# mishapadidar/GP-Derivatives-Variational-Inference

Hardware: AMD Instinct MI355X
Metric: ELBO steps/sec, DSVGP d=20 N=1M M=500 p=5 (higher is better)
Workload: dtype f32 (f64 Cholesky/solves); 1 GPU; DSVGP d=20 N=1M M=500 p=5 B=4096; global_batch=4096, per_gpu_batch=4096, M_prime=3000, parallelism=dp1 rows, trsm_nb=4096, graph_replay=False, one_call_step=True, dense_product=hand-written (gemm32.hip, v_mfma_f32_32x32x2_f32)

## Files before the change

gp-derivatives-variational-inference_amd/csrc/common.h:

```cpp
#pragma once
#include <hip/hip_runtime.h>
#include <stdint.h>
#include <stdio.h>

#include "dsvgp.h"

struct dsvgp_ctx {
    hipStream_t stream = nullptr;
    void* blas = nullptr;
    void* det_slab = nullptr;
    size_t det_bytes = 0;
    bool prezeroed = false;
    bool lean_classic = false;
    bool fwd_lower_only = false;
    struct PointsJob { const float* slab; int ns; const float* partials; int nparts; float sym; };
    bool defer_points = false;
    int n_deferred = 0;
    PointsJob deferred[2];
};

#define DSVGP_LAUNCH_CHECK()                                  \
    do {                                                      \
        hipError_t e__ = hipGetLastError();                   \
        if (e__ != hipSuccess) return 1000 + (int)e__;        \
// ... 29 lines not shown
constexpr int DSVGP_GEMM_KEEP_UPPER = 1 << 20;
constexpr int DSVGP_GEMM_C_ZEROED = 1 << 21;
constexpr int DSVGP_GEMM_UPPER_UNDEF = 1 << 22;
int launch_gemm(hipStream_t st, int is_double, const GemmArgs& g);
hipError_t zero_block(void* C, size_t esz, int64_t ld, int M, int N, hipStream_t st);
void launch_cvt_f64_f32(hipStream_t st, const double* C, int64_t ldc, float* C32, int64_t ldc32, int M, int N);
void launch_widen_f32_f64(hipStream_t st, const float* src, int64_t ld, double* dst, int64_t ldd, int M, int N);
int launch_gemm64(hipStream_t st, const GemmArgs& g);
int launch_gemm32(hipStream_t st, const GemmArgs& g);

int launch_det_sum_rows64(hipStream_t st, const double* parts, int ns, int64_t n, double* out);
int launch_det_sum_scalars64(hipStream_t st, const double* parts, int n, int nc, double* out);
static inline double* det_scratch64(const dsvgp_ctx* ctx, size_t doubles) {
    return (ctx->det_slab && ctx->det_bytes / sizeof(double) >= doubles && ((uintptr_t)ctx->det_slab % 8) == 0) ? (double*)ctx->det_slab : nullptr;
}
static inline int bwd64_tiled_sweep(int ntr, int ntc, int* nsg) {
    int sweep = (int)(((int64_t)ntr * ntc) / 1024);
    sweep = sweep < 32 ? sweep : 32;
    sweep = sweep < ntc ? sweep : ntc;
    sweep = sweep > 1 ? sweep : 1;
    *nsg = cdiv(ntc, sweep);
    return sweep;
}
size_t kernel_bwd64_tiled_det_bytes(int n1, int n2, int d, int p);

size_t potrf_blocked_workspace_bytes(int n);
struct PotrfHook { int after_k; hipEvent_t ev; };
int launch_potrf_blocked(hipStream_t st, double* A, int n, int64_t lda, int* info, double* ws, double* Yinv, int64_t ldy,
                         double* YinvT, bool info_zeroed = false, const PotrfHook* hooks = nullptr, int nhooks = 0, int pipe_from = 0);
int launch_pack_both(hipStream_t st, const float* Z, const float* V, int M, const float* X, const float* D, int B, int d, int p,
                     const float* rl, const float* rs, const float* rn, float* hyp, float* center, float* PZ, float* sZ, float* vZ,
                     float* PX, float* sX, float* vX);
int kernel_bwd_points_flush(dsvgp_ctx* ctx, const float* P1, const float* vnorm1, int n1, int d, int p, const float* hyp, float* d_x1,
                            float* d_v1, float* d_hyp, const float* scal, const float* kl0, double rows, double num_data, const float* rl,
                            const float* rs, const float* rn, float* drl, float* drs, float* drn, float* dconst, float* loss);
int launch_column_mean_hyp(hipStream_t st, const float* x, int n, int d, float* center, const float* rl, const float* rs,
                           const float* rn, float* hyp);
int launch_kernel_fwd_wide(hipStream_t st, const float* P1, const float* self1, int n1q, const float* P2, const float* self2, int n2q,
                           int q, int K4, int DP, const float* hyp, float jitter, void* out, int64_t ld, int out_is_double);
size_t kernel_bwd_wide_workspace(int n1q, int n2q, int q, int NP);
int launch_kernel_bwd_wide(hipStream_t st, const void* G, int64_t ldg, int g_is_double, const float* P1, const float* self1, int n1q,
                           const float* P2, const float* self2, int n2q, int q, int K4, int DP, int NP, const float* hyp, void* workspace,
                           float** slab, int* ns, float** partials, int* nparts);
int launch_widen_sym_f32_f64(hipStream_t st, const float* src, int64_t lds, double* dst, int64_t ldd, int n);
int launch_mirror_sminus_i_col(hipStream_t st, float* A, int n, int64_t lda, const float* m, const float* hyp, float rows, double* W = nullptr,
                               int64_t ldw = 0);
int launch_variational_terms(hipStream_t st, const float* m, const float* LS, int64_t ldls, int Mp, double num_data, int flags,
                             const float* hyp, double global_rows, const float* G, int64_t ldg, float t1_scale, float* kl_out,
                             float* sums, const float* dm_src, float* d_m, float* d_LS, int64_t lddls, int fin_npts, int fin_p,
                             float* fin_scal);
int launch_stats_residual(dsvgp_ctx* ctx, const float* A, int64_t lda, int Mp, int ncols, int p, const float* m,
                          const float* constant, const float* hyp, float* mu, float* var, void* workspace, const float* y,
                          double global_rows, float* mu_bar, float* sums);
int launch_scale_epilogue(dsvgp_ctx* ctx, float* x0, int64_t n0, float* x1, int64_t n1, const float* hyp, double rows,
                          const float* scal, const float* kl0, double num_data, const float* rl, const float* rs, const float* rn,
                          float* dh, float* drl, float* drs, float* drn, float* dconst, float* loss);

int launch_trtri_blocks(hipStream_t st, const double* L, int64_t ldl, int n, int nb, double* Dinv,
                        int64_t ldd, double* tmp, const double* X64);
```

gp-derivatives-variational-inference_amd/csrc/elbo.hip:

```cpp
#include "common.h"

namespace {

constexpr float KXX_JITTER = 1e-4f;
constexpr float NOISE_FLOOR = 1e-4f;
constexpr float MIN_VARIANCE = 1e-6f;

__device__ __forceinline__ float softplusf(float x) { return x > 20.f ? x : log1pf(expf(x)); }
__device__ __forceinline__ float sigmoidf(float x) { return 1.f / (1.f + expf(-x)); }

__global__ void hyp_forward_kernel(const float* rl, const float* rs, const float* rn, float* hyp) {
    if (threadIdx.x == 0) {
        hyp[0] = softplusf(rl[0]);
        hyp[1] = softplusf(rs[0]);
        hyp[2] = softplusf(rn[0]) + NOISE_FLOOR;
        hyp[3] = 0.f;
    }
}
__global__ void hyp_backward_kernel(const float* rl, const float* rs, const float* rn, const float* dh, float* drl,
                                    float* drs, float* drn) {
    if (threadIdx.x == 0) {
        drl[0] += dh[0] * sigmoidf(rl[0]);
        drs[0] += dh[1] * sigmoidf(rs[0]);
        drn[0] += dh[2] * sigmoidf(rn[0]);
    }
}

__global__ void step_epilogue_kernel(const float* scal, const float* kl0, float inv_rows, float inv_num_data,
                                     const float* rl, const float* rs, const float* rn, float* dh, float* drl,
                                     float* drs, float* drn, float* dconst, float* loss) {
    if (threadIdx.x == 0) {
        const float d0 = dh[0] + scal[4], d1 = dh[1] + scal[3], d2 = dh[2] + scal[1];
        dh[0] = d0; dh[1] = d1; dh[2] = d2;
        drl[0] += d0 * sigmoidf(rl[0]);
        drs[0] += d1 * sigmoidf(rs[0]);
        drn[0] += d2 * sigmoidf(rn[0]);
        dconst[0] += scal[2];
        loss[0] = -scal[0] * inv_rows + kl0[0] * inv_num_data;
    }
}

__global__ __launch_bounds__(256) void colstats_kernel(const float* __restrict__ A, int64_t lda,
                                                       const float* __restrict__ W, int64_t ldw, int Mp, int ncols,
                                                       const float* __restrict__ m, int rows_per_chunk,
                                                       float* __restrict__ part) {
    const int j = blockIdx.x * 256 + threadIdx.x;
    const int i0 = blockIdx.y * rows_per_chunk, i1 = min(Mp, i0 + rows_per_chunk);
    if (j >= ncols) return;
    float sm = 0.f, sq = 0.f;
    if (W == A) {
#pragma unroll 4
        for (int i = i0; i < i1; ++i) sm = fmaf(A[(int64_t)i * lda + j], m[i], sm);
    } else {
        for (int i = i0; i < i1; ++i) {
            const float a = A[(int64_t)i * lda + j], w = W[(int64_t)i * ldw + j];
            sm = fmaf(a, m[i], sm);
            sq += w * w - a * a;
        }
    }
    part[((int64_t)blockIdx.y * 2) * ncols + j] = sm;
    part[((int64_t)blockIdx.y * 2 + 1) * ncols + j] = sq;
}
__global__ void colstats_finish_kernel(const float* __restrict__ part, int nchunk, int ncols, int p,
                                       const float* __restrict__ constant, const float* __restrict__ hyp,
                                       float* __restrict__ mu, float* __restrict__ var) {
    const int j = blockIdx.x * blockDim.x + threadIdx.x;
    if (j >= ncols) return;
    float sm = 0.f, sq = 0.f;
    for (int c = 0; c < nchunk; ++c) {
        sm += part[((int64_t)c * 2) * ncols + j];
        sq += part[((int64_t)c * 2 + 1) * ncols + j];
    }
    const float ell = hyp[0], s = hyp[1];
    const float dg = (j % (p + 1) == 0) ? s : s / (ell * ell);
    mu[j] = sm + constant[0];
    var[j] = dg + KXX_JITTER + sq;
}

__global__ __launch_bounds__(256) void likelihood_kernel(const float* __restrict__ mu, const float* __restrict__ var,
                                                         const float* __restrict__ y, int ncols, int p,
                                                         const float* __restrict__ hyp, int mll_type, float inv_rows,
                                                         float* __restrict__ mu_bar, float* __restrict__ var_bar,
                                                         float* __restrict__ varn_out, float* __restrict__ scal, float* __restrict__ partials) {
    __shared__ float red[5][4];
    const float ell = hyp[0], s = hyp[1], noise = hyp[2];
    const float LOG2PI = 1.8378770664093453f;
    float acc[5] = {0.f, 0.f, 0.f, 0.f, 0.f};
    for (int j = blockIdx.x * 256 + threadIdx.x; j < ncols; j += gridDim.x * 256) {
        const float mj = mu[j], r = y[j] - mj;
        const float vraw = var[j] + noise;
        const bool clamped = vraw < MIN_VARIANCE;
        const float vn = clamped ? MIN_VARIANCE : vraw;
        float ll, dmu, dvn, dnoise;
        if (mll_type == 0) {
            ll = -0.5f * ((r * r + vn) / noise + logf(noise) + LOG2PI);
            dmu = r / noise;
            dvn = -0.5f / noise;
            dnoise = 0.5f * (r * r + vn) / (noise * noise) - 0.5f / noise;
        } else {
            const float tot = fmaxf(vn + noise, 1e-8f);
            ll = -0.5f * (r * r / tot + logf(tot) + LOG2PI);
            dmu = r / tot;
            dvn = 0.5f * (r * r / (tot * tot) - 1.f / tot);
            dnoise = dvn;
        }
        const float dvar = clamped ? 0.f : dvn;
        dnoise += dvar;
        const float mb = -dmu * inv_rows, vb = -dvar * inv_rows;
        mu_bar[j] = mb;
        var_bar[j] = vb;
        varn_out[j] = vn;
        const bool isf = (j % (p + 1)) == 0;
        acc[0] += ll;
        acc[1] += -dnoise * inv_rows;
// ... 800 lines not shown
                                             float* const* exp_avgs, float* const* exp_avg_sqs, const int64_t* sizes, float lr,
                                             float beta1, float beta2, float eps, int step, const int* guard_dev) {
    return adam_step_multi_impl(ctx, count, params, grads, exp_avgs, exp_avg_sqs, sizes, lr, beta1, beta2, eps, step, guard_dev);
}
static int adam_step_multi_impl(dsvgp_ctx* ctx, int count, float* const* params, const float* const* grads, float* const* exp_avgs,
                                float* const* exp_avg_sqs, const int64_t* sizes, float lr, float beta1, float beta2, float eps, int step,
                                const int* guard_dev) {
    if (!ctx || count < 0 || count > DSVGP_ADAM_MAX_TENSORS || step < 1) return DSVGP_EINVAL;
    if (count && (!params || !grads || !exp_avgs || !exp_avg_sqs || !sizes)) return DSVGP_EINVAL;
    AdamTable t{};
    int nblocks = 0;
    for (int k = 0; k < count; ++k) {
        if (sizes[k] != 0 && (!params[k] || !grads[k] || !exp_avgs[k] || !exp_avg_sqs[k])) return DSVGP_EINVAL;
        if (sizes[k] == 0) continue;
        const int c = t.count++;
        t.param[c] = params[k]; t.grad[c] = grads[k]; t.m[c] = exp_avgs[k]; t.v[c] = exp_avg_sqs[k]; t.n[c] = sizes[k];
        int b = sizes[k] < 0 ? (int)(-sizes[k] < 2048 ? -sizes[k] : 2048) : cdiv(sizes[k], 256);
        if (b > 2048) b = 2048;
        t.first[c] = nblocks;
        nblocks += b;
    }
    if (!t.count) return 0;
    t.first[t.count] = nblocks;
    const double bc1 = 1.0 - pow((double)beta1, step), bc2 = 1.0 - pow((double)beta2, step);
    hipLaunchKernelGGL(adam_multi_kernel, dim3(nblocks), dim3(256), 0, ctx->stream, t, lr, beta1, beta2, eps, (float)bc1,
                       (float)sqrt(bc2), guard_dev);
    DSVGP_LAUNCH_CHECK();
    return 0;
}

int launch_stats_residual(dsvgp_ctx* ctx, const float* A, int64_t lda, int Mp, int ncols, int p, const float* m,
                          const float* constant, const float* hyp, float* mu, float* var, void* workspace, const float* y,
                          double global_rows, float* mu_bar, float* sums) {
    if (ctx->det_slab || ncols == 0) {
        int rc = dsvgp_predictive_stats(ctx, A, lda, A, lda, Mp, ncols, p, m, constant, hyp, mu, var, workspace);
        if (rc) return rc;
        return dsvgp_residual_terms(ctx, mu, y, ncols, hyp, global_rows, mu_bar, sums);
    }
    if (!ctx->prezeroed) {
        hipError_t e = hipMemsetAsync(sums, 0, 4 * sizeof(float), ctx->stream);
        if (e != hipSuccess) return 1000 + (int)e;
    }
    const int nch = stats_chunks(Mp), rpc = cdiv(Mp, nch);
    hipLaunchKernelGGL(colstats_kernel, dim3(cdiv(ncols, 256), nch), dim3(256), 0, ctx->stream, A, lda, A, lda, Mp, ncols, m, rpc,
                       (float*)workspace);
    DSVGP_LAUNCH_CHECK();
    int blocks = cdiv(ncols, 256);
    if (blocks > 512) blocks = 512;
    hipLaunchKernelGGL(colstats_residual_kernel, dim3(blocks), dim3(256), 0, ctx->stream, (const float*)workspace, nch, ncols, p,
                       constant, hyp, mu, var, y, (float)(1.0 / global_rows), mu_bar, sums);
    DSVGP_LAUNCH_CHECK();
    return 0;
}
int launch_scale_epilogue(dsvgp_ctx* ctx, float* x0, int64_t n0, float* x1, int64_t n1, const float* hyp, double rows,
                          const float* scal, const float* kl0, double num_data, const float* rl, const float* rs, const float* rn,
                          float* dh, float* drl, float* drs, float* drn, float* dconst, float* loss) {
    const int64_t tot = n0 + n1;
    int blocks = (int)((tot + 255) / 256);
    if (blocks < 1) blocks = 1;
    if (blocks > 2048) blocks = 2048;
    hipLaunchKernelGGL(scale_epilogue_kernel, dim3(blocks), dim3(256), 0, ctx->stream, x0, n0, x1, n1, hyp, (float)(1.0 / rows), scal,
                       kl0, (float)(1.0 / num_data), rl, rs, rn, dh, drl, drs, drn, dconst, loss);
    DSVGP_LAUNCH_CHECK();
    return 0;
}

extern "C" int dsvgp_residual_terms(dsvgp_ctx* ctx, const float* mu, const float* y, int ncols, const float* hyp,
                                    double global_rows, float* mu_bar, float* sums) {
    if (!ctx || !mu || !y || !hyp || !mu_bar || !sums || ncols < 0 || global_rows <= 0) return DSVGP_EINVAL;
    if (!ctx->prezeroed) {
        hipError_t e = hipMemsetAsync(sums, 0, 4 * sizeof(float), ctx->stream);
        if (e != hipSuccess) return 1000 + (int)e;
    }
    if (ncols == 0) return 0;
    int blocks = cdiv(ncols, 256);
    if (blocks > 512) blocks = 512;
    float* partials = (ctx->det_slab && ctx->det_bytes >= (size_t)blocks * 8 * sizeof(float)) ? (float*)ctx->det_slab : nullptr;
    hipLaunchKernelGGL(residual_kernel, dim3(blocks), dim3(256), 0, ctx->stream, mu, y, ncols, hyp,
                       (float)(1.0 / global_rows), mu_bar, sums, partials);
    DSVGP_LAUNCH_CHECK();
    if (partials) {
        hipLaunchKernelGGL(partials_reduce_kernel, dim3(1), dim3(64), 0, ctx->stream, (const float*)partials, blocks, 2, sums);
        DSVGP_LAUNCH_CHECK();
    }
    return 0;
}
extern "C" int dsvgp_trace_terms(dsvgp_ctx* ctx, const float* LS, int64_t ldls, const float* T1, int64_t ldt,
                                 const float* G, int64_t ldg, int n, float t1_scale, float* sums) {
    if (!ctx || !LS || !T1 || !G || !sums || n <= 0) return DSVGP_EINVAL;
    hipLaunchKernelGGL(trace_kernel, dim3(n < 1024 ? n : 1024), dim3(256), 0, ctx->stream, LS, ldls, T1, ldt, G, ldg, n, t1_scale, sums);
    DSVGP_LAUNCH_CHECK();
    return 0;
}
extern "C" int dsvgp_elbo_fast_finalize(dsvgp_ctx* ctx, const float* sums, const float* hyp, int npts, int p,
                                        double global_rows, float* out_scalars) {
    if (!ctx || !sums || !hyp || !out_scalars || npts < 0 || p < 0 || global_rows <= 0) return DSVGP_EINVAL;
    hipLaunchKernelGGL(elbo_fast_finalize_kernel, dim3(1), dim3(64), 0, ctx->stream, sums, hyp, npts, p,
                       (float)(1.0 / global_rows), out_scalars);
    DSVGP_LAUNCH_CHECK();
    return 0;
}
extern "C" int dsvgp_mirror_lower_f32(dsvgp_ctx* ctx, float* G, int n, int64_t ldg) {
    if (!ctx || !G || n <= 0 || ldg < n) return DSVGP_EINVAL;
    const int nb = cdiv(n, 32);
    hipLaunchKernelGGL(mirror_lower_f32_kernel, dim3(nb, nb), dim3(32, 8), 0, ctx->stream, G, n, ldg);
    DSVGP_LAUNCH_CHECK();
// ... 155 lines not shown
```

gp-derivatives-variational-inference_amd/csrc/step.hip:

```cpp
#include "common.h"

#include <stdlib.h>
#include <string.h>

#include <new>

namespace {

struct Carve {
    size_t off = 0;
    size_t take(size_t bytes) {
        const size_t o = off;
        off += (bytes + 255) / 256 * 256;
        return o;
    }
};

inline int pad4(int n) { return (n + 3) / 4 * 4; }
inline int auto_nb(int Mp) {
    int b = 64;
    while (b < Mp) b <<= 1;
    return b;
}

}

struct dsvgp_step_plan {
    int M, d, p, B, Mp, Bp, DP, nb;
    bool per_output = false;
    size_t o_A64 = 0, o_U32 = 0, o_Abar = 0, o_Kb64 = 0, o_var = 0, o_varbar = 0;
    int world = 1;
    int wq = 0, wr = 0;
    size_t o_Qfull = 0, o_qcol64 = 0, o_cbT = 0, o_cbK = 0, o_slab = 0, slab_bytes = 0, o_lrow64 = 0;
    hipEvent_t ev_dp = nullptr;
    size_t bytes;
    size_t o_zero, zero_bytes;
    size_t o_info, o_sums, o_klbuf, o_scal, o_hyp, o_center;
    size_t o_PZ, o_sZ, o_vZ, o_PX, o_sX, o_vX;
    size_t o_phi32 = 0; bool phi32_own = false;
    bool precleared_ge = false;
    bool precleared = false;
    size_t o_L, o_trsm, o_potrf, o_Kzx, o_A32e, o_S32e, o_var0, o_stats, o_Ge, o_Qe64, o_S64e, o_Qe32, o_Kb32, o_G1, o_Yt, o_Kbar, o_kbwd, o_kbwd2;
    size_t o_arena, arena_bytes;
    int ldS, ldQ32;
    const void* pad_ready_for = nullptr;
    hipStream_t side = nullptr;
    hipEvent_t ev_fork = nullptr, ev_side = nullptr, ev_status = nullptr, ev_fork2 = nullptr, ev_var = nullptr, ev_dense = nullptr,
               ev_zx = nullptr, ev_pipe1 = nullptr, ev_pipe2 = nullptr, ev_s = nullptr;
    static constexpr int TM_RING = 128, TM_PAIRS = 5;
    hipEvent_t tm_ring[TM_RING][2 * TM_PAIRS] = {};
    hipEvent_t* tm = tm_ring[0];
    long timed_steps = 0;
    bool timed = false;
    float* host_status = nullptr;
};

#ifndef STEP_S_LATE
#define STEP_S_LATE 2
#define STEP_S_LATE_MP 1024
#endif
static size_t step_layout(int M, int d, int p, int B, dsvgp_step_plan* pl, int world = 1) {
    if (M <= 0 || d <= 0 || p < 0 || B <= 0 || world < 1 || world > 64 || (world > 1 && M < world)) return 0;
    const int q = p + 1, Mp = M * q, Bp = B * q, DP = dsvgp_packed_width(d);
    if (DP <= 0 || Mp > 8192 || (int64_t)Mp * Bp >= ((int64_t)1 << 31)) return 0;
    pl->M = M; pl->d = d; pl->p = p; pl->B = B; pl->Mp = Mp; pl->Bp = Bp; pl->DP = DP; pl->nb = auto_nb(Mp);
    pl->ldS = pad4(Mp + 1); pl->ldQ32 = pad4(Mp + 1);
    Carve c;
    pl->o_scal = c.take(8 * sizeof(float)); pl->o_center = c.take((size_t)d * sizeof(float));
    pl->o_PZ = c.take((size_t)Mp * DP * 4); pl->o_sZ = c.take((size_t)Mp * 4); pl->o_vZ = c.take((size_t)(M * p > 0 ? M * p : 1) * 4);
    pl->o_PX = c.take((size_t)Bp * DP * 4); pl->o_sX = c.take((size_t)Bp * 4); pl->o_vX = c.take((size_t)(B * p > 0 ? B * p : 1) * 4);
    pl->o_L = c.take((size_t)Mp * Mp * 8);
    pl->o_potrf = c.take(potrf_blocked_workspace_bytes(Mp));
    pl->o_Kzx = c.take((size_t)Mp * Bp * 4); pl->o_A32e = c.take((size_t)(Mp + 1) * Bp * 4);
    pl->o_var0 = c.take((size_t)Bp * 4); pl->o_stats = c.take(dsvgp_stats_workspace_bytes(Mp, Bp) + 16);
    pl->o_Qe32 = c.take((size_t)Mp * pl->ldQ32 * 4);
    pl->o_S64e = c.take((size_t)(Mp + 1) * ((Mp + 1) / 2 * 2) * 8);
    const size_t kb = dsvgp_kernel_bwd_workspace_bytes(M, B, d, p), kz = dsvgp_kernel_bwd_workspace_bytes(M, M, d, p);
    pl->o_kbwd = c.take(kb > kz ? kb : kz); pl->o_kbwd2 = c.take(kb);
    const int nrhs_max = Bp > Mp + 1 ? Bp : Mp + 1;
    const size_t trsm_bytes = dsvgp_trsm_workspace_bytes(Mp, nrhs_max, pl->nb);
    pl->o_trsm = c.take(trsm_bytes);
    pl->o_arena = (pl->o_trsm + sizeof(double) * ((size_t)2 * Mp * Mp + (size_t)(Mp + pl->nb) * (pl->nb / 2))) / 256 * 256;
    pl->o_S32e = c.take((size_t)Mp * pl->ldS * 4);
    pl->o_Ge = c.take((size_t)(Mp + 1) * Mp * 4); pl->o_Qe64 = c.take((size_t)Mp * (Mp + 2) * 8 + 64);
    pl->o_Kb32 = c.take((size_t)Mp * Bp * 4); pl->o_G1 = c.take((size_t)Mp * Mp * 8);
    pl->o_Yt = c.take((size_t)Mp * Mp * 8); pl->o_Kbar = c.take((size_t)Mp * Mp * 8);
    pl->phi32_own = true;
    pl->o_phi32 = c.take((size_t)Mp * pl->ldQ32 * 4);
    pl->o_zero = c.off;
    pl->zero_bytes = (4 * sizeof(float) + 4 * sizeof(int) + 4 * sizeof(float) + (size_t)(2 * Mp + 1) * sizeof(float) + 255) / 256 * 256;
    pl->o_hyp = c.take(pl->zero_bytes);
    pl->o_info = pl->o_hyp + 4 * sizeof(float);
    pl->o_sums = pl->o_info + 4 * sizeof(int);
    pl->o_klbuf = pl->o_sums + 4 * sizeof(float);
    pl->arena_bytes = c.off - pl->o_arena;
    pl->world = world;
    if (world > 1) {
        const int q1 = p + 1;
        pl->wq = ((Mp + 1 + world - 1) / world + 3) / 4 * 4;
        pl->wr = ((Mp + world - 1) / world + 1) / 2 * 2;
        const int wc = ((M + world - 1) / world) * q1;
        pl->o_Qfull = c.take((size_t)Mp * world * pl->wq * 4);
        pl->o_qcol64 = c.take((size_t)Mp * pl->wq * 8);
        pl->o_lrow64 = c.take((size_t)pl->wr * Mp * 8);
        pl->o_cbT = c.take((size_t)Mp * wc * 8);
        pl->o_cbK = c.take((size_t)Mp * wc * 8);
        pl->slab_bytes = (size_t)4 * Mp * Mp * 4 + 4096;
        pl->o_slab = c.take(pl->slab_bytes);
    }
    if (pl->per_output) {
        pl->o_A64 = c.take((size_t)Mp * Bp * 8);
        pl->o_U32 = c.take((size_t)Mp * Bp * 4);
        pl->o_Abar = c.take((size_t)Mp * Bp * 4);
        pl->o_Kb64 = c.take((size_t)Mp * Bp * 8);
        pl->o_var = c.take((size_t)Bp * 4);
        pl->o_varbar = c.take((size_t)Bp * 4);
    }
    pl->bytes = c.off + 256;
    return pl->bytes;
}

static size_t split_offsets(int Mp, int Bp, size_t* o_pat, size_t* o_pq) {
    size_t off = (dsvgp_split3_bytes(Mp + 1, Bp) + 255) / 256 * 256;
    if (o_pat) *o_pat = off;
    off += (dsvgp_split3_bytes(Bp, Mp + 1) + 255) / 256 * 256;
    if (o_pq) *o_pq = off;
    off += (dsvgp_split3_bytes(Mp, Mp + 1) + 255) / 256 * 256;
    return off;
}
extern "C" size_t dsvgp_elbo_step_split_bytes(int M, int d, int p, int B) {
    if (M <= 0 || d <= 0 || p < 0 || B <= 0) return 0;
    return split_offsets(M * (p + 1), B * (p + 1), nullptr, nullptr);
}

extern "C" size_t dsvgp_elbo_step_workspace_bytes(int M, int d, int p, int B) {
    dsvgp_step_plan pl{};
    return step_layout(M, d, p, B, &pl);
}

extern "C" size_t dsvgp_elbo_step_dp_workspace_bytes(int M, int d, int p, int B, int world) {
    dsvgp_step_plan pl{};
    return step_layout(M, d, p, B, &pl, world);
}

static int plan_create(dsvgp_ctx* ctx, int M, int d, int p, int B, int world, dsvgp_step_plan** out, bool per_output = false) {
    if (!ctx || !out) return DSVGP_EINVAL;
    dsvgp_step_plan* pl = new (std::nothrow) dsvgp_step_plan();
    if (!pl) return DSVGP_EINVAL;
    pl->per_output = per_output;
    if (!step_layout(M, d, p, B, pl, world)) { delete pl; return DSVGP_EINVAL; }
    bool ok = hipStreamCreateWithFlags(&pl->side, hipStreamNonBlocking) == hipSuccess;
    hipEvent_t* evs[] = {&pl->ev_fork, &pl->ev_side, &pl->ev_status, &pl->ev_fork2, &pl->ev_var, &pl->ev_dense, &pl->ev_zx, &pl->ev_dp,
                         &pl->ev_pipe1, &pl->ev_pipe2, &pl->ev_s};
    for (hipEvent_t* e : evs) ok = ok && hipEventCreateWithFlags(e, hipEventDisableTiming) == hipSuccess;
    for (auto& slot : pl->tm_ring) for (hipEvent_t& e : slot) ok = ok && hipEventCreate(&e) == hipSuccess;
    ok = ok && hipHostMalloc((void**)&pl->host_status, 8 * sizeof(float), hipHostMallocDefault) == hipSuccess;
    if (!ok) {
        (void)hipGetLastError();
        for (hipEvent_t* e : evs) if (*e) (void)hipEventDestroy(*e);
        for (auto& slot : pl->tm_ring) for (hipEvent_t e : slot) if (e) (void)hipEventDestroy(e);
        if (pl->side) (void)hipStreamDestroy(pl->side);
        if (pl->host_status) (void)hipHostFree(pl->host_status);
        delete pl;
        return 1000 + (int)hipErrorOutOfMemory;
    }
    pl->host_status[4] = 0.f;
    *out = pl;
    return 0;
}
extern "C" int dsvgp_elbo_step_plan_create(dsvgp_ctx* ctx, int M, int d, int p, int B, dsvgp_step_plan** out) {
    return plan_create(ctx, M, d, p, B, 1, out);
}
extern "C" int dsvgp_elbo_step_dp_plan_create(dsvgp_ctx* ctx, int M, int d, int p, int B, int world, dsvgp_step_plan** out) {
    if (world < 2) return DSVGP_EINVAL;
    return plan_create(ctx, M, d, p, B, world, out);
}

extern "C" int dsvgp_elbo_step_po_plan_create(dsvgp_ctx* ctx, int M, int d, int p, int B, dsvgp_step_plan** out) {
    return plan_create(ctx, M, d, p, B, 1, out, true);
}
extern "C" size_t dsvgp_elbo_step_po_workspace_bytes(int M, int d, int p, int B) {
    dsvgp_step_plan pl{};
    pl.per_output = true;
    return step_layout(M, d, p, B, &pl);
}

extern "C" int dsvgp_elbo_step_plan_destroy(dsvgp_step_plan* pl) {
    if (!pl) return DSVGP_EINVAL;
    hipEvent_t evs[] = {pl->ev_fork, pl->ev_side, pl->ev_status, pl->ev_fork2, pl->ev_var, pl->ev_dense, pl->ev_zx, pl->ev_dp, pl->ev_pipe1,
                        pl->ev_pipe2, pl->ev_s};
    for (hipEvent_t e : evs) if (e) (void)hipEventDestroy(e);
    for (auto& slot : pl->tm_ring) for (hipEvent_t e : slot) if (e) (void)hipEventDestroy(e);
    if (pl->side) (void)hipStreamDestroy(pl->side);
    if (pl->host_status) (void)hipHostFree(pl->host_status);
    delete pl;
    return 0;
}

static int step_timings(dsvgp_step_plan* pl, int back, float* ms, int n) {
    if (!pl || !ms || n < 1 || n > dsvgp_step_plan::TM_PAIRS || back < 0 || back >= dsvgp_step_plan::TM_RING || back >= pl->timed_steps)
        return DSVGP_EINVAL;
    hipEvent_t* tm = pl->tm_ring[(pl->timed_steps - 1 - back) % dsvgp_step_plan::TM_RING];
    for (int k = 0; k < n; ++k) {
        hipError_t e = hipEventSynchronize(tm[2 * k + 1]);
        if (e == hipSuccess) e = hipEventElapsedTime(&ms[k], tm[2 * k], tm[2 * k + 1]);
        if (e != hipSuccess) return 1000 + (int)e;
    }
    return 0;
}
extern "C" int dsvgp_elbo_step_timings(dsvgp_step_plan* pl, int back, float* ms3) { return step_timings(pl, back, ms3, 3); }
extern "C" int dsvgp_elbo_step_timings5(dsvgp_step_plan* pl, int back, float* ms5) { return step_timings(pl, back, ms5, 5); }

extern "C" size_t dsvgp_elbo_step_plan_bytes(const dsvgp_step_plan* pl) { return pl ? pl->bytes : 0; }
extern "C" long dsvgp_elbo_step_timed_count(const dsvgp_step_plan* pl) { return pl ? pl->timed_steps : 0; }

extern "C" int dsvgp_elbo_step_locate(const dsvgp_step_plan* pl, int which, size_t* offset_bytes, int* rows, int* cols, int64_t* ld) {
    if (!pl || !offset_bytes || !rows || !cols || !ld) return DSVGP_EINVAL;
    switch (which) {
        case 0: *offset_bytes = pl->o_A32e; *rows = pl->Mp + 1; *cols = pl->Bp; *ld = pl->Bp; return 0;
        case 1: *offset_bytes = pl->o_Kzx; *rows = pl->Mp; *cols = pl->Bp; *ld = pl->Bp; return 0;
        case 2: *offset_bytes = pl->o_L; *rows = pl->Mp; *cols = pl->Mp; *ld = pl->Mp; return 0;
        case 3: *offset_bytes = pl->o_trsm; *rows = pl->Mp; *cols = pl->Mp; *ld = pl->Mp; return 0;
        case 4: *offset_bytes = pl->o_hyp; *rows = 1; *cols = 4; *ld = 4; return 0;
        case 5: *offset_bytes = pl->o_info; *rows = 1; *cols = 1; *ld = 1; return 0;
        default: return DSVGP_EINVAL;
    }
}

extern "C" int dsvgp_elbo_step_status(dsvgp_step_plan* pl, float* hyp4, int* info) {
    if (!pl || !info) return DSVGP_EINVAL;
    hipError_t e = hipEventSynchronize(pl->ev_status);
    if (e != hipSuccess) return 1000 + (int)e;
    if (hyp4) for (int i = 0; i < 4; ++i) hyp4[i] = pl->host_status[i];
    int v;
    memcpy(&v, &pl->host_status[4], sizeof(int));
    *info = v;
    return 0;
}

#ifndef STEP_VAR_LATE_MP
#define STEP_VAR_LATE_MP 1536
#endif
#ifndef STEP_Q_CLASSIC_BP
// ... 36 lines not shown
    if (zz_canon2(io, d, p) && rows_in_16_byte_pieces(Kbar, ld, 8))
        return dsvgp_kernel_bwd_canon2(ctx, Kbar, ld, 1, PZ, vZ, M, P2, n2, d, p, io->dir_idx, io->dir_idx_base, hyp, 1, io->dZ, io->dV,
                                       io->d_hyp, ws);
    return dsvgp_kernel_bwd(ctx, Kbar, ld, 1, PZ, sZ, vZ, M, P2, s2, n2, d, p, hyp, 1, io->dZ, io->dV, io->d_hyp, ws);
}
static int zx_fwd(dsvgp_ctx* ctx, const dsvgp_elbo_step_io* io, const float* PZ, const float* sZ, int M, const float* PX, const float* sX,
                  int B, int d, int p, const float* hyp, float* Kzx, int64_t ld) {
    if (zz_canon2(io, d, p)) return dsvgp_kernel_fwd_canon2(ctx, PZ, M, PX, B, d, p, io->dir_idx, io->dir_idx_base, hyp, 0.f, Kzx, ld, 0);
    if (zx_canon(io, d, p)) return dsvgp_kernel_fwd_canon(ctx, PZ, sZ, M, PX, sX, B, d, p, io->dir_idx, io->dir_idx_base, hyp, Kzx, ld);
    return dsvgp_kernel_fwd(ctx, PZ, sZ, M, PX, sX, B, d, p, hyp, 0.f, Kzx, ld, 0);
}
static int zx_bwd(dsvgp_ctx* ctx, const dsvgp_elbo_step_io* io, const float* Kb32, int64_t ld, const float* PZ, const float* sZ,
                  const float* vZ, int M, const float* PX, const float* sX, int B, int d, int p, const float* hyp, void* ws) {
    if (zz_canon2(io, d, p) && rows_in_16_byte_pieces(Kb32, ld, 4))
        return dsvgp_kernel_bwd_canon2(ctx, Kb32, ld, 0, PZ, vZ, M, PX, B, d, p, io->dir_idx, io->dir_idx_base, hyp, 0, io->dZ, io->dV,
                                       io->d_hyp, ws);
    if (zx_canon(io, d, p))
        return dsvgp_kernel_bwd_canon(ctx, Kb32, ld, 0, PZ, sZ, vZ, M, PX, sX, B, d, p, io->dir_idx, io->dir_idx_base, hyp, io->dZ, io->dV,
                                      io->d_hyp, ws);
    return dsvgp_kernel_bwd(ctx, Kb32, ld, 0, PZ, sZ, vZ, M, PX, sX, B, d, p, hyp, 0, io->dZ, io->dV, io->d_hyp, ws);
}

static int step_validate(dsvgp_ctx* ctx, dsvgp_step_plan* pl, const dsvgp_elbo_step_io* io, void* workspace, size_t workspace_bytes) {
    if (!ctx || !pl || !io || !workspace || workspace_bytes < pl->bytes || ((uintptr_t)workspace % 256)) return DSVGP_EINVAL;
    if (!io->Z || !io->m || !io->LS || !io->constant || !io->raw_lengthscale || !io->raw_outputscale || !io->raw_noise || !io->x ||
        !io->y || !io->flat || !io->dZ || !io->dm || !io->dLS || !io->d_hyp || !io->d_constant || !io->d_raw_lengthscale ||
        !io->d_raw_outputscale || !io->d_raw_noise || !io->loss || !io->mu || io->num_data <= 0 || io->global_rows <= 0)
        return DSVGP_EINVAL;
    const int p = pl->p, Mp = pl->Mp;
    if (p > 0 && (!io->V || !io->D || !io->dV)) return DSVGP_EINVAL;
    if (io->ldls < Mp || io->lddls < Mp) return DSVGP_EINVAL;
    return 0;
}

#define STEP_LOCALS \
    [[maybe_unused]] const int M = pl->M, d = pl->d, p = pl->p, B = pl->B, Mp = pl->Mp, Bp = pl->Bp, nb = pl->nb; \
    [[maybe_unused]] char* w = (char*)workspace; \
    [[maybe_unused]] int* info = (int*)(w + pl->o_info); \
    [[maybe_unused]] float* sums = (float*)(w + pl->o_sums); \
    [[maybe_unused]] float* kl_buf = (float*)(w + pl->o_klbuf); \
    [[maybe_unused]] float* scal = (float*)(w + pl->o_scal); \
    [[maybe_unused]] float* hyp = (float*)(w + pl->o_hyp); \
    [[maybe_unused]] float* center = (float*)(w + pl->o_center); \
    [[maybe_unused]] float *PZ = (float*)(w + pl->o_PZ), *sZ = (float*)(w + pl->o_sZ), *vZ = (float*)(w + pl->o_vZ); \
    [[maybe_unused]] float *PX = (float*)(w + pl->o_PX), *sX = (float*)(w + pl->o_sX), *vX = (float*)(w + pl->o_vX); \
    [[maybe_unused]] double* L = (double*)(w + pl->o_L); \
    [[maybe_unused]] void* trsm_ws = w + pl->o_trsm; \
    [[maybe_unused]] void* potrf_ws = w + pl->o_potrf; \
    [[maybe_unused]] float* Kzx = (float*)(w + pl->o_Kzx); \
    [[maybe_unused]] float* A32e = (float*)(w + pl->o_A32e); \
    [[maybe_unused]] float* S32e = (float*)(w + pl->o_S32e); \
    [[maybe_unused]] float* var0 = (float*)(w + pl->o_var0); \
    [[maybe_unused]] void* stats_ws = w + pl->o_stats; \
    [[maybe_unused]] float* Ge = (float*)(w + pl->o_Ge); \
    [[maybe_unused]] double* Qe64 = (double*)(w + pl->o_Qe64); \
    [[maybe_unused]] double* S64e = (double*)(w + pl->o_S64e); \
    [[maybe_unused]] float* Qe32 = (float*)(w + pl->o_Qe32); \
    [[maybe_unused]] float* Kb32 = (float*)(w + pl->o_Kb32); \
    [[maybe_unused]] double* G1 = (double*)(w + pl->o_G1); \
    [[maybe_unused]] double* Yt = (double*)(w + pl->o_Yt); \
    [[maybe_unused]] double* Kbar = (double*)(w + pl->o_Kbar); \
    [[maybe_unused]] void* kbwd_ws = w + pl->o_kbwd; \
    [[maybe_unused]] void* kbwd_ws2 = w + pl->o_kbwd2; \
    [[maybe_unused]] const int ldS = pl->ldS, ldQ32 = pl->ldQ32, ldQ64 = (Mp + 2) / 2 * 2, ldST = (Mp + 1) / 2 * 2; \
    [[maybe_unused]] const double rows = io->global_rows;

struct ZeroedScope {
    dsvgp_ctx* c; bool prev;
    ZeroedScope(dsvgp_ctx* c_, bool on) : c(c_), prev(c_->prezeroed) { if (on) c->prezeroed = true; }
    ~ZeroedScope() { c->prezeroed = prev; }
};
static int step_front(dsvgp_ctx* ctx, dsvgp_step_plan* pl, const dsvgp_elbo_step_io* io, void* workspace, int flags, bool preclear = false) {
    STEP_LOCALS
    const bool overlap = (flags & 1) && !ctx->det_slab;
    const bool timed = flags & 4;
    pl->timed = timed;
    if (timed) { pl->tm = pl->tm_ring[pl->timed_steps % dsvgp_step_plan::TM_RING]; ++pl->timed_steps; }
#define STEP_TIME(slot) do { if (timed) STEP_HIP(hipEventRecord(pl->tm[slot], ctx->stream)); } while (0)
    const hipStream_t main = ctx->stream, side = pl->side;

    const bool prezero = pl->arena_bytes <= ((size_t)48 << 20) && !ctx->det_slab;
    static const bool preclear_env = !getenv("DSVGP_PRECLEAR") || atoi(getenv("DSVGP_PRECLEAR")) != 0;
    pl->precleared = preclear && preclear_env && overlap && !prezero && !ctx->det_slab && !(flags & (16 | 32 | 64));
    pl->precleared_ge = false;
    STEP_HIP(hipMemsetAsync(io->flat, 0, io->flat_floats * sizeof(float), main));
    if (prezero) STEP_HIP(hipMemsetAsync(w + pl->o_arena, 0, pl->arena_bytes, main));
    else STEP_HIP(hipMemsetAsync(w + pl->o_zero, 0, pl->zero_bytes, main));
    if (pl->pad_ready_for != workspace || (flags & 8)) {
        STEP_HIP(hipMemsetAsync(Qe32, 0, (size_t)Mp * ldQ32 * sizeof(float), main));
        STEP_HIP(hipMemsetAsync(S32e, 0, (size_t)Mp * ldS * sizeof(float), main));
        pl->pad_ready_for = workspace;
    }
    struct PrezeroGuard {
        dsvgp_ctx* c; bool prev;
        PrezeroGuard(dsvgp_ctx* c_, bool on) : c(c_), prev(c_->prezeroed) { c->prezeroed = on; }
        ~PrezeroGuard() { c->prezeroed = prev; }
    } prezero_guard(ctx, prezero);
    STEP_CALL(launch_pack_both(main, io->Z, io->V, M, io->x, io->D, B, d, p, io->raw_lengthscale, io->raw_outputscale, io->raw_noise, hyp,
                               center, PZ, sZ, vZ, PX, sX, vX));
    static const int s_late_env = getenv("DSVGP_S_LATE") ? atoi(getenv("DSVGP_S_LATE")) : -1;
    const int s_late = !overlap ? 0 : s_late_env >= 0 ? s_late_env : (Mp >= STEP_S_LATE_MP ? STEP_S_LATE : 0);
    auto prologue_s = [&](bool background) -> int {
        int rc = dsvgp_gemm(ctx, 0, DSVGP_GEMM_A_LOWER | DSVGP_GEMM_TRANS_B | DSVGP_GEMM_B_UPPER | DSVGP_GEMM_OUT_LOWER |
                            (background ? DSVGP_GEMM_BACKGROUND : 0), Mp, Mp, Mp, 1.0, io->LS, io->ldls, io->LS, io->ldls, 0.0, nullptr, 0,
                            S32e, ldS, nullptr, 0, nullptr);
        if (rc) return rc;
        rc = launch_mirror_sminus_i_col(ctx->stream, S32e, Mp, ldS, io->m, hyp, (float)rows, S64e, ldST);
        if (rc) return rc;
        const hipError_t e = hipGetLastError();
        return e == hipSuccess ? 0 : 1000 + (int)e;
    };
    auto prologue = [&](bool background) -> int {
        int rc = 0;
        if (timed && hipEventRecord(pl->tm[2], ctx->stream) != hipSuccess) return 1000 + (int)hipGetLastError();
        rc = zx_fwd(ctx, io, PZ, sZ, M, PX, sX, B, d, p, hyp, Kzx, Bp);
        if (rc) return rc;
        if (timed && hipEventRecord(pl->tm[3], ctx->stream) != hipSuccess) return 1000 + (int)hipGetLastError();
        if (s_late) return 0;
        return prologue_s(background);
    };
    float* A32 = A32e;
    float* mu_bar = A32e + (size_t)Mp * Bp;
    static const int pipe_k1 = getenv("DSVGP_PIPE_K1") ? atoi(getenv("DSVGP_PIPE_K1")) : STEP_PIPE_K1;
    static const int pipe_k2 = getenv("DSVGP_PIPE_K2") ? atoi(getenv("DSVGP_PIPE_K2")) : STEP_PIPE_K2;
    static const int pipe_pad = getenv("DSVGP_PIPE_PAD") ? atoi(getenv("DSVGP_PIPE_PAD")) : STEP_PIPE_PAD;
    const int nblk64 = (Mp + 63) / 64;
    const int pk1 = (int)((int64_t)nblk64 * pipe_k1 / 1000), pk2 = (int)((int64_t)nblk64 * pipe_k2 / 1000);
    const bool pipe = overlap && (flags & 128) && nb >= Mp && Mp % 2 == 0 && Bp % 4 == 0 && ((uintptr_t)Kzx % 16) == 0 &&
                      (int64_t)nblk64 * ((Bp + 63) / 64) >= 8192 && nblk64 >= 16 && pipe_k1 >= 0 && pk1 <= pk2 && pk2 <= nblk64 - 2 &&
                      pipe_pad >= 0 && pipe_pad <= 98304;
    const double* LinvT = (const double*)trsm_ws + (size_t)Mp * Mp;
    auto solve_rows = [&](int ra, int rb, int pad) -> int {
        GemmArgs f{};
        f.batch = 1; f.splitk = 1;
        f.M = rb - ra; f.N = Bp; f.K = rb; f.tri_off = ra; f.wide64 = 1; f.lds_pad = pad;
        f.A = LinvT + ra; f.lda = Mp; f.flags = DSVGP_GEMM_TRANS_A | DSVGP_GEMM_A_LOWER | DSVGP_GEMM_B_IS_FLOAT;
        f.B = Kzx; f.ldb = Bp; f.alpha = 1.0; f.beta = 0.0;
        f.C = nullptr; f.C32 = A32 + (size_t)ra * Bp; f.ldc32 = Bp;
        return launch_gemm(ctx->stream, 1, f);
    };
    int r2 = 0;
    if (overlap) STEP_HIP(hipEventRecord(pl->ev_fork, main));
    STEP_CALL(zz_fwd(ctx, io, PZ, sZ, M, d, p, hyp, L, Mp));
    auto clear_tail_targets = [&]() -> int {
        STEP_HIP(hipMemsetAsync(Yt, 0, (size_t)Mp * Mp * sizeof(double), side));
        STEP_HIP(hipMemsetAsync(Kbar, 0, (size_t)Mp * Mp * sizeof(double), side));
        STEP_HIP(hipMemsetAsync(w + pl->o_phi32, 0, (size_t)Mp * ldQ32 * sizeof(float), side));
        return 0;
    };
    auto side_prologue = [&]() -> int {
        if (!overlap) return 0;
        STEP_HIP(hipStreamWaitEvent(side, pl->ev_fork, 0));
        if (pl->precleared && !s_late) {
            STEP_CALL(clear_tail_targets());
            STEP_HIP(hipMemsetAsync(Ge, 0, (size_t)(Mp + 1) * Mp * sizeof(float), side));
            pl->precleared_ge = true;
        }
        ctx->stream = side;
        const int rc = prologue(true);
        ctx->stream = main;
        if (rc) return rc;
        STEP_HIP(hipEventRecord(pl->ev_side, side));
        return 0;
    };
    if (pipe) {
        const int k1 = pk1, k2 = pk2;
        const int r1 = (k1 + 1) * 64;
        r2 = (k2 + 1) * 64;
        const PotrfHook hooks[2] = {{k1, pl->ev_pipe1}, {k2, pl->ev_pipe2}};
        double* Dinv = (double*)trsm_ws;
        STEP_CALL(launch_potrf_blocked(main, L, Mp, Mp, info, (double*)potrf_ws, Dinv, Mp, Dinv + (size_t)Mp * Mp, ctx->prezeroed, hooks,
                                       k2 > k1 ? 2 : 1));
        STEP_CALL(side_prologue());
        ctx->stream = side;
        STEP_HIP(hipStreamWaitEvent(side, pl->ev_pipe1, 0));
        STEP_TIME(0);
        STEP_CALL(solve_rows(0, r1, pipe_pad));
        if (k2 > k1) {
            STEP_HIP(hipStreamWaitEvent(side, pl->ev_pipe2, 0));
            STEP_CALL(solve_rows(r1, r2, pipe_pad));
        } else r2 = r1;
        STEP_TIME(1);
        STEP_HIP(hipEventRecord(pl->ev_pipe1, side));
        ctx->stream = main;
    } else {
        STEP_CALL(dsvgp_potrf_inverse(ctx, L, Mp, Mp, info, potrf_ws, nb, trsm_ws));
        STEP_CALL(side_prologue());
    }
    if (overlap) {
        STEP_HIP(hipStreamWaitEvent(main, pl->ev_side, 0));
        STEP_HIP(hipEventRecord(pl->ev_fork2, main));
        STEP_HIP(hipStreamWaitEvent(side, pl->ev_fork2, 0));
        STEP_HIP(hipMemcpyAsync(pl->host_status, hyp, 5 * sizeof(float), hipMemcpyDeviceToHost, side));
        STEP_HIP(hipEventRecord(pl->ev_status, side));
        if (s_late) {
            if (pl->precleared) STEP_CALL(clear_tail_targets());
            ctx->stream = side;
            const int rc = prologue_s(s_late == 1);
            ctx->stream = main;
            if (rc) return rc;
            STEP_HIP(hipEventRecord(pl->ev_s, side));
        }
    } else {
        STEP_HIP(hipMemcpyAsync(pl->host_status, hyp, 5 * sizeof(float), hipMemcpyDeviceToHost, main));
        STEP_HIP(hipEventRecord(pl->ev_status, main));
        STEP_CALL(prologue(false));
    }
    if (pipe) {
        STEP_CALL(solve_rows(r2, Mp, 0));
        STEP_HIP(hipStreamWaitEvent(main, pl->ev_pipe1, 0));
    } else {
        STEP_TIME(0);
        STEP_CALL(dsvgp_trsm(ctx, L, Mp, Mp, 0, Kzx, Bp, 0, Bp, nullptr, 0, A32, Bp, nb, trsm_ws, 1));
        STEP_TIME(1);
    }
    STEP_CALL(launch_stats_residual(ctx, A32, Bp, Mp, Bp, p, io->m, io->constant, hyp, io->mu, var0, stats_ws, io->y, rows, mu_bar, sums));
    STEP_TIME(6);
    if (flags & 32) {
        if (!io->split_ws || ((uintptr_t)io->split_ws & 255) || io->split_ws_bytes < split_offsets(Mp, Bp, nullptr, nullptr)) {
            ctx->stream = main;
            return DSVGP_EINVAL;
        }
        STEP_CALL(dsvgp_split3_bf16(ctx, A32e, Bp, Mp + 1, Bp, 0, io->split_ws));
        STEP_CALL(dsvgp_gemm3b(ctx, DSVGP_GEMM_OUT_LOWER, Mp + 1, Mp, Bp, 1.f, io->split_ws, Mp + 1, io->split_ws, Mp + 1, Ge, Mp));
    } else {
        ZeroedScope zs(ctx, pl->precleared_ge);
        STEP_CALL(dsvgp_gemm(ctx, 0, DSVGP_GEMM_TRANS_B | DSVGP_GEMM_OUT_LOWER, Mp + 1, Mp, Bp, 1.0, A32e, Bp, A32, Bp, 0.0, nullptr, 0, Ge,
                             Mp, nullptr, 0, nullptr));
    }
    STEP_TIME(7);
    if (s_late) STEP_HIP(hipStreamWaitEvent(main, pl->ev_s, 0));
    return 0;
}

extern "C" int dsvgp_elbo_step_f32(dsvgp_ctx* ctx, dsvgp_step_plan* pl, const dsvgp_elbo_step_io* io, void* workspace,
                                   size_t workspace_bytes, int flags) {
    if (int rc = step_validate(ctx, pl, io, workspace, workspace_bytes)) return rc;
    if (pl->world != 1) return DSVGP_EINVAL;
    STEP_LOCALS
    const bool overlap = (flags & 1) && !ctx->det_slab;
    const bool include_kl = flags & 2, timed = flags & 4;
    const hipStream_t main = ctx->stream, side = pl->side;
    struct PrezeroGuard {
        dsvgp_ctx* c; bool prev;
        PrezeroGuard(dsvgp_ctx* c_, bool on) : c(c_), prev(c_->prezeroed) { c->prezeroed = on; }
        ~PrezeroGuard() { c->prezeroed = prev; }
    } prezero_guard(ctx, pl->arena_bytes <= ((size_t)48 << 20) && !ctx->det_slab);
    STEP_CALL(step_front(ctx, pl, io, workspace, flags, true));
    STEP_CALL(dsvgp_mirror_lower_f32(ctx, Ge, Mp, Mp));
    auto variational = [&]() -> int {
        int rc = dsvgp_gemm(ctx, 0, DSVGP_GEMM_B_LOWER | DSVGP_GEMM_OUT_LOWER, Mp, Mp, Mp, 1.0, Ge, Mp, io->LS, io->ldls, 0.0, nullptr, 0,
                            io->dLS, io->lddls, nullptr, 0, nullptr);
        if (rc) return rc;
        return launch_variational_terms(ctx->stream, io->m, io->LS, io->ldls, Mp, io->num_data, 1 | (include_kl ? 2 : 0), hyp, rows, Ge, Mp,
                                        1.f, kl_buf, sums, Ge + (size_t)Mp * Mp, io->dm, io->dLS, io->lddls, B, p, scal);
    };
    const bool var_late = overlap && !(flags & 16) && Mp >= STEP_VAR_LATE_MP;
    auto solve_q = [&]() -> int {
        const bool small = (int64_t)((Mp + 63) / 64) * ((Mp + 1 + 63) / 64) < 1024;
        const bool prev = ctx->lean_classic;
        ctx->lean_classic = overlap && !var_late && Bp >= STEP_Q_CLASSIC_BP;
        const int rc = dsvgp_trsm(ctx, L, Mp, Mp, 1, S32e, ldS, 0, Mp + 1, small ? Qe64 : nullptr, ldQ64, Qe32, ldQ32, nb, trsm_ws, 1);
        ctx->lean_classic = prev;
        return rc;
    };
    auto dense_product = [&]() -> int {
        if (flags & 32) {
            size_t o_pat, o_pq;
            split_offsets(Mp, Bp, &o_pat, &o_pq);
// ... 319 lines not shown
```

Measured before the change: 83.49 steps/s.

## Compute predictive mean from LinvT·m on side stream, overlapping the triangular solve

Adds a path that computes the predictive mean without waiting for the large triangular solve. It first forms w = L^{-T} m in fp64, then takes column dot products of Kzx with w, and runs both on the side stream while the main stream runs the TRSM. The main stream then waits on an event instead of launching the stats/residual kernel over A32. The Ge clear is also moved onto the side stream. Separately, the Cholesky info buffer is treated as pre-zeroed by default, which skips a clear. The risks are an extra full read of Kzx competing with the solve for bandwidth, and the variance partials now being written as zero, so correctness depends on var being computed elsewhere.

```diff
diff --git a/gp-derivatives-variational-inference_amd/csrc/common.h b/gp-derivatives-variational-inference_amd/csrc/common.h
--- a/gp-derivatives-variational-inference_amd/csrc/common.h
+++ b/gp-derivatives-variational-inference_amd/csrc/common.h
@@ -105,6 +105,9 @@
 int launch_stats_residual(dsvgp_ctx* ctx, const float* A, int64_t lda, int Mp, int ncols, int p, const float* m,
                           const float* constant, const float* hyp, float* mu, float* var, void* workspace, const float* y,
                           double global_rows, float* mu_bar, float* sums);
+int launch_mean_residual_w(hipStream_t st, const double* LinvT, int64_t ldl, const float* Kzx, int64_t ldk, int Mp, int ncols, int p,
+                           const float* m, const float* constant, const float* hyp, float* mu, float* var, void* workspace, double* wvec,
+                           const float* y, double global_rows, float* mu_bar, float* sums);
 int launch_scale_epilogue(dsvgp_ctx* ctx, float* x0, int64_t n0, float* x1, int64_t n1, const float* hyp, double rows,
                           const float* scal, const float* kl0, double num_data, const float* rl, const float* rs, const float* rn,
                           float* dh, float* drl, float* drs, float* drn, float* dconst, float* loss);
diff --git a/gp-derivatives-variational-inference_amd/csrc/elbo.hip b/gp-derivatives-variational-inference_amd/csrc/elbo.hip
--- a/gp-derivatives-variational-inference_amd/csrc/elbo.hip
+++ b/gp-derivatives-variational-inference_amd/csrc/elbo.hip
@@ -60,6 +60,36 @@
     }
     part[((int64_t)blockIdx.y * 2) * ncols + j] = sm;
     part[((int64_t)blockIdx.y * 2 + 1) * ncols + j] = sq;
+}
+__global__ __launch_bounds__(256) void linvt_m_kernel(const double* __restrict__ LinvT, int64_t ld, int n, const float* __restrict__ m,
+                                                      double* __restrict__ w) {
+    const int j = blockIdx.x * 4 + (threadIdx.x >> 6), lane = threadIdx.x & 63;
+    if (j >= n) return;
+    const double* __restrict__ r = LinvT + (int64_t)j * ld;
+    double s = 0.0;
+    for (int i = j + lane; i < n; i += 64) s = fma(r[i], (double)m[i], s);
+    for (int off = 32; off > 0; off >>= 1) s += __shfl_down(s, off);
+    if (lane == 0) w[j] = s;
+}
+__global__ __launch_bounds__(256) void colmean_w_kernel(const float* __restrict__ K, int64_t ldk, int Mp, int ncols,
+                                                        const double* __restrict__ w, int rows_per_chunk, float* __restrict__ part) {
+    __shared__ double ws[256];
+    const int j = blockIdx.x * 256 + threadIdx.x;
+    const int i0 = blockIdx.y * rows_per_chunk, i1 = min(Mp, i0 + rows_per_chunk);
+    double s = 0.0;
+    for (int b = i0; b < i1; b += 256) {
+        const int nb = min(256, i1 - b);
+        __syncthreads();
+        if ((int)threadIdx.x < nb) ws[threadIdx.x] = w[b + threadIdx.x];
+        __syncthreads();
+        if (j < ncols) {
+#pragma unroll 4
+            for (int i = 0; i < nb; ++i) s = fma((double)K[(int64_t)(b + i) * ldk + j], ws[i], s);
+        }
+    }
+    if (j >= ncols) return;
+    part[((int64_t)blockIdx.y * 2) * ncols + j] = (float)s;
+    part[((int64_t)blockIdx.y * 2 + 1) * ncols + j] = 0.f;
 }
 __global__ void colstats_finish_kernel(const float* __restrict__ part, int nchunk, int ncols, int p,
                                        const float* __restrict__ constant, const float* __restrict__ hyp,
@@ -966,6 +996,22 @@
     DSVGP_LAUNCH_CHECK();
     return 0;
 }
+int launch_mean_residual_w(hipStream_t st, const double* LinvT, int64_t ldl, const float* Kzx, int64_t ldk, int Mp, int ncols, int p,
+                           const float* m, const float* constant, const float* hyp, float* mu, float* var, void* workspace, double* wvec,
+                           const float* y, double global_rows, float* mu_bar, float* sums) {
+    hipLaunchKernelGGL(linvt_m_kernel, dim3(cdiv(Mp, 4)), dim3(256), 0, st, LinvT, ldl, Mp, m, wvec);
+    DSVGP_LAUNCH_CHECK();
+    const int nch = stats_chunks(Mp), rpc = cdiv(Mp, nch);
+    hipLaunchKernelGGL(colmean_w_kernel, dim3(cdiv(ncols, 256), nch), dim3(256), 0, st, Kzx, ldk, Mp, ncols, (const double*)wvec, rpc,
+                       (float*)workspace);
+    DSVGP_LAUNCH_CHECK();
+    int blocks = cdiv(ncols, 256);
+    if (blocks > 512) blocks = 512;
+    hipLaunchKernelGGL(colstats_residual_kernel, dim3(blocks), dim3(256), 0, st, (const float*)workspace, nch, ncols, p, constant, hyp, mu,
+                       var, y, (float)(1.0 / global_rows), mu_bar, sums);
+    DSVGP_LAUNCH_CHECK();
+    return 0;
+}
 int launch_scale_epilogue(dsvgp_ctx* ctx, float* x0, int64_t n0, float* x1, int64_t n1, const float* hyp, double rows,
                           const float* scal, const float* kl0, double num_data, const float* rl, const float* rs, const float* rn,
                           float* dh, float* drl, float* drs, float* drn, float* dconst, float* loss) {
diff --git a/gp-derivatives-variational-inference_amd/csrc/step.hip b/gp-derivatives-variational-inference_amd/csrc/step.hip
--- a/gp-derivatives-variational-inference_amd/csrc/step.hip
+++ b/gp-derivatives-variational-inference_amd/csrc/step.hip
@@ -40,11 +40,13 @@
     size_t o_phi32 = 0; bool phi32_own = false;
     bool precleared_ge = false;
     bool precleared = false;
+    size_t o_wvec = 0;
     size_t o_L, o_trsm, o_potrf, o_Kzx, o_A32e, o_S32e, o_var0, o_stats, o_Ge, o_Qe64, o_S64e, o_Qe32, o_Kb32, o_G1, o_Yt, o_Kbar, o_kbwd, o_kbwd2;
     size_t o_arena, arena_bytes;
     int ldS, ldQ32;
     const void* pad_ready_for = nullptr;
     hipStream_t side = nullptr;
+    hipEvent_t ev_mean = nullptr;
     hipEvent_t ev_fork = nullptr, ev_side = nullptr, ev_status = nullptr, ev_fork2 = nullptr, ev_var = nullptr, ev_dense = nullptr,
                ev_zx = nullptr, ev_pipe1 = nullptr, ev_pipe2 = nullptr, ev_s = nullptr;
     static constexpr int TM_RING = 128, TM_PAIRS = 5;
@@ -73,6 +75,7 @@
     pl->o_potrf = c.take(potrf_blocked_workspace_bytes(Mp));
     pl->o_Kzx = c.take((size_t)Mp * Bp * 4); pl->o_A32e = c.take((size_t)(Mp + 1) * Bp * 4);
     pl->o_var0 = c.take((size_t)Bp * 4); pl->o_stats = c.take(dsvgp_stats_workspace_bytes(Mp, Bp) + 16);
+    pl->o_wvec = c.take((size_t)Mp * 8);
     pl->o_Qe32 = c.take((size_t)Mp * pl->ldQ32 * 4);
     pl->o_S64e = c.take((size_t)(Mp + 1) * ((Mp + 1) / 2 * 2) * 8);
     const size_t kb = dsvgp_kernel_bwd_workspace_bytes(M, B, d, p), kz = dsvgp_kernel_bwd_workspace_bytes(M, M, d, p);
@@ -143,6 +146,10 @@
     return step_layout(M, d, p, B, &pl, world);
 }
 
+#ifndef STEP_MEAN_SIDE_MP
+#define STEP_MEAN_SIDE_MP 1024
+#endif
+
 static int plan_create(dsvgp_ctx* ctx, int M, int d, int p, int B, int world, dsvgp_step_plan** out, bool per_output = false) {
     if (!ctx || !out) return DSVGP_EINVAL;
     dsvgp_step_plan* pl = new (std::nothrow) dsvgp_step_plan();
@@ -151,7 +158,7 @@
     if (!step_layout(M, d, p, B, pl, world)) { delete pl; return DSVGP_EINVAL; }
     bool ok = hipStreamCreateWithFlags(&pl->side, hipStreamNonBlocking) == hipSuccess;
     hipEvent_t* evs[] = {&pl->ev_fork, &pl->ev_side, &pl->ev_status, &pl->ev_fork2, &pl->ev_var, &pl->ev_dense, &pl->ev_zx, &pl->ev_dp,
-                         &pl->ev_pipe1, &pl->ev_pipe2, &pl->ev_s};
+                         &pl->ev_pipe1, &pl->ev_pipe2, &pl->ev_s, &pl->ev_mean};
     for (hipEvent_t* e : evs) ok = ok && hipEventCreateWithFlags(e, hipEventDisableTiming) == hipSuccess;
     for (auto& slot : pl->tm_ring) for (hipEvent_t& e : slot) ok = ok && hipEventCreate(&e) == hipSuccess;
     ok = ok && hipHostMalloc((void**)&pl->host_status, 8 * sizeof(float), hipHostMallocDefault) == hipSuccess;
@@ -188,7 +195,7 @@
 extern "C" int dsvgp_elbo_step_plan_destroy(dsvgp_step_plan* pl) {
     if (!pl) return DSVGP_EINVAL;
     hipEvent_t evs[] = {pl->ev_fork, pl->ev_side, pl->ev_status, pl->ev_fork2, pl->ev_var, pl->ev_dense, pl->ev_zx, pl->ev_dp, pl->ev_pipe1,
-                        pl->ev_pipe2, pl->ev_s};
+                        pl->ev_pipe2, pl->ev_s, pl->ev_mean};
     for (hipEvent_t e : evs) if (e) (void)hipEventDestroy(e);
     for (auto& slot : pl->tm_ring) for (hipEvent_t e : slot) if (e) (void)hipEventDestroy(e);
     if (pl->side) (void)hipStreamDestroy(pl->side);
@@ -331,6 +338,7 @@
     [[maybe_unused]] float* S32e = (float*)(w + pl->o_S32e); \
     [[maybe_unused]] float* var0 = (float*)(w + pl->o_var0); \
     [[maybe_unused]] void* stats_ws = w + pl->o_stats; \
+    [[maybe_unused]] double* wvec = (double*)(w + pl->o_wvec); \
     [[maybe_unused]] float* Ge = (float*)(w + pl->o_Ge); \
     [[maybe_unused]] double* Qe64 = (double*)(w + pl->o_Qe64); \
     [[maybe_unused]] double* S64e = (double*)(w + pl->o_S64e); \
@@ -419,6 +427,9 @@
         return launch_gemm(ctx->stream, 1, f);
     };
     int r2 = 0;
+    static const bool info_fold = !getenv("DSVGP_INFO_FOLD") || atoi(getenv("DSVGP_INFO_FOLD")) != 0;
+    static const int mean_side_env = getenv("DSVGP_MEAN_SIDE") ? atoi(getenv("DSVGP_MEAN_SIDE")) : -1;
+    const bool mean_side = overlap && Bp > 0 && (mean_side_env >= 0 ? mean_side_env != 0 : Mp >= STEP_MEAN_SIDE_MP);
     if (overlap) STEP_HIP(hipEventRecord(pl->ev_fork, main));
     STEP_CALL(zz_fwd(ctx, io, PZ, sZ, M, d, p, hyp, L, Mp));
     auto clear_tail_targets = [&]() -> int {
@@ -448,7 +459,7 @@
         r2 = (k2 + 1) * 64;
         const PotrfHook hooks[2] = {{k1, pl->ev_pipe1}, {k2, pl->ev_pipe2}};
         double* Dinv = (double*)trsm_ws;
-        STEP_CALL(launch_potrf_blocked(main, L, Mp, Mp, info, (double*)potrf_ws, Dinv, Mp, Dinv + (size_t)Mp * Mp, ctx->prezeroed, hooks,
+        STEP_CALL(launch_potrf_blocked(main, L, Mp, Mp, info, (double*)potrf_ws, Dinv, Mp, Dinv + (size_t)Mp * Mp, ctx->prezeroed || info_fold, hooks,
                                        k2 > k1 ? 2 : 1));
         STEP_CALL(side_prologue());
         ctx->stream = side;
@@ -463,21 +474,34 @@
         STEP_HIP(hipEventRecord(pl->ev_pipe1, side));
         ctx->stream = main;
     } else {
-        STEP_CALL(dsvgp_potrf_inverse(ctx, L, Mp, Mp, info, potrf_ws, nb, trsm_ws));
+        {
+            ZeroedScope zs(ctx, info_fold);
+            STEP_CALL(dsvgp_potrf_inverse(ctx, L, Mp, Mp, info, potrf_ws, nb, trsm_ws));
+        }
         STEP_CALL(side_prologue());
     }
     if (overlap) {
         STEP_HIP(hipStreamWaitEvent(main, pl->ev_side, 0));
         STEP_HIP(hipEventRecord(pl->ev_fork2, main));
         STEP_HIP(hipStreamWaitEvent(side, pl->ev_fork2, 0));
+        if (mean_side) {
+            STEP_CALL(launch_mean_residual_w(side, LinvT, Mp, Kzx, Bp, Mp, Bp, p, io->m, io->constant, hyp, io->mu, var0, stats_ws, wvec, io->y,
+                                             rows, mu_bar, sums));
+            if (!(flags & 32) && !pl->precleared_ge) {
+                STEP_HIP(hipMemsetAsync(Ge, 0, (size_t)(Mp + 1) * Mp * sizeof(float), side));
+                pl->precleared_ge = true;
+            }
+            STEP_HIP(hipEventRecord(pl->ev_mean, side));
+        }
         STEP_HIP(hipMemcpyAsync(pl->host_status, hyp, 5 * sizeof(float), hipMemcpyDeviceToHost, side));
         STEP_HIP(hipEventRecord(pl->ev_status, side));
         if (s_late) {
-            if (pl->precleared) STEP_CALL(clear_tail_targets());
+            if (pl->precleared && !mean_side) STEP_CALL(clear_tail_targets());
             ctx->stream = side;
             const int rc = prologue_s(s_late == 1);
             ctx->stream = main;
             if (rc) return rc;
+            if (pl->precleared && mean_side) STEP_CALL(clear_tail_targets());
             STEP_HIP(hipEventRecord(pl->ev_s, side));
         }
     } else {
@@ -493,7 +517,8 @@
         STEP_CALL(dsvgp_trsm(ctx, L, Mp, Mp, 0, Kzx, Bp, 0, Bp, nullptr, 0, A32, Bp, nb, trsm_ws, 1));
         STEP_TIME(1);
     }
-    STEP_CALL(launch_stats_residual(ctx, A32, Bp, Mp, Bp, p, io->m, io->constant, hyp, io->mu, var0, stats_ws, io->y, rows, mu_bar, sums));
+    if (mean_side) STEP_HIP(hipStreamWaitEvent(main, pl->ev_mean, 0));
+    else STEP_CALL(launch_stats_residual(ctx, A32, Bp, Mp, Bp, p, io->m, io->constant, hyp, io->mu, var0, stats_ws, io->y, rows, mu_bar, sums));
     STEP_TIME(6);
     if (flags & 32) {
         if (!io->split_ws || ((uintptr_t)io->split_ws & 255) || io->split_ws_bytes < split_offsets(Mp, Bp, nullptr, nullptr)) {
```

Result: no change. 83.04 steps/s (-0.5%).
